# mrluin/TextualDegRemoval

Measured on AMD Instinct MI355X. Metric: train images/sec (512x512, bs=4/GPU), higher is better.
Workload: dtype f32 (3xbf16-split MFMA: 24-bit operand significands on the full fp32 exponent range, fp32 accumulate; unscaled gradients, no loss scale, no step-skip guard; tensors fp32 -- the MASA-encoder ResidualBlock activations / gradients as three bf16 planes whose sum IS the fp32 value, bit for bit)

## Files before the change

### include/tdr.h

```cpp
#ifndef TDR_H
#define TDR_H
#include <stdint.h>
#ifdef __cplusplus
extern "C" {
#endif

#define TDR_ABI_VERSION 109
int tdr_version(void);
const char* tdr_last_error(void);

typedef struct TdrStepGuard {
    float scale, inv_scale, max_scale;
    int good, growth_interval;
    int step, skipped, finite;
    float bc1, bc2_sqrt;
} TdrStepGuard;

typedef struct TdrConvDesc {
    int N, Cin, H, W;
    int Cout, OH, OW;
    int KH, stride, dil, pad;
    const float* in;  int64_t in_ns;
    int gate;
    const float* kscale; int64_t kscale_ns;
// ... 74 lines not shown
    float* g;
    float* db;
    int per_image;
    float* ws; int64_t ws_floats;
    int math;
} TdrWgradDesc;
int64_t tdr_wgrad_ws_floats(const TdrWgradDesc* d);
int tdr_conv_wgrad(const TdrWgradDesc* d, void* stream);

typedef struct TdrWg1GroupEntry {
    const float* in; const float* dout; float* part; float* dbpart; float* g; float* db;
} TdrWg1GroupEntry;
int tdr_wgrad1x1_group_supported(const TdrWgradDesc* d);
int64_t tdr_wgrad1x1_group_ws_floats(const TdrWgradDesc* d, int nprob);
int tdr_wgrad1x1_group(const TdrWgradDesc* d, int nprob, const void* table, void* stream);

int tdr_layernorm2d_fwd(const float* x, int64_t x_ns, const float* w, const float* b, float eps, int center,
                        int N, int C, int HW, float* y, float* mu, float* rstd, void* stream);
int64_t tdr_ln_ws_floats(int N, int C, int HW);
int tdr_layernorm2d_bwd(const float* go, const float* x, int64_t x_ns, const float* mu, const float* rstd,
                        const float* w, const float* add, int64_t add_ns, int add_C, int center,
                        int N, int C, int HW, float* gx, float* gw, float* gb, float* ws, void* stream);

int64_t tdr_dwsg_ws_floats(int N, int C, int H, int W);
int tdr_dwsg_fwd(const float* t, const float* w, const float* b, int N, int C, int H, int W,
                 float* g, float* pooled, float* ws, void* stream);
int tdr_dwsg_bwd(const float* dg, const float* t, const float* w, const float* b, int N, int C, int H, int W,
                 float* dt, float* dw, float* db, float* ws, void* stream);
int tdr_dwsg_bwd_biased(const float* dg, const float* dg_bias, float dg_bias_mul, const float* t, const float* w, const float* b,
                        int N, int C, int H, int W, float* dt, float* dw, float* db, float* ws, void* stream);
// ... 364 lines not shown
```

### textualdegremoval_amd/_lib.py

```python
import ctypes as C
import os

import torch

_HERE = os.path.dirname(os.path.abspath(__file__))
LIB_PATH = os.environ.get('TDR_LIB_PATH', os.path.join(_HERE, 'libtdr_hip.so'))

ABI_VERSION = 109
c_fp = C.c_void_p
i32, i64, f32 = C.c_int, C.c_int64, C.c_float


class TdrConvDesc(C.Structure):
    _fields_ = [
        ('N', i32), ('Cin', i32), ('H', i32), ('W', i32),
        ('Cout', i32), ('OH', i32), ('OW', i32),
        ('KH', i32), ('stride', i32), ('dil', i32), ('pad', i32),
        ('inp', c_fp), ('in_ns', i64),
        ('gate', i32),
        ('kscale', c_fp), ('kscale_ns', i64),
        ('wp', c_fp), ('wp_ns', i64), ('Mpad', i32), ('wp_fmt', i32),
        ('out', c_fp), ('out_ns', i64),
        ('epi', i32),
        ('bias', c_fp), ('bias_ns', i64),
# ... 115 lines not shown
    'tdr_conv3x3_p16_force_cfg': (i32, [i32]),
    'tdr_wgrad3x3_p16_ws_floats': (i64, [C.POINTER(TdrWgradP16Desc)]),
    'tdr_wgrad3x3_p16': (i32, [C.POINTER(TdrWgradP16Desc), c_fp]),
    'tdr_packed_weight_floats': (i64, [i32, i32, i32]),
    'tdr_pack_weights': (i32, [c_fp, i32, i32, i32, i32, c_fp, c_fp]),
    'tdr_packed_weight_bytes_bx3': (i64, [i32, i32, i32]),
    'tdr_pack_weights_bx3': (i32, [c_fp, i32, i32, i32, i32, c_fp, c_fp]),
    'tdr_pack_job_init': (i32, [C.POINTER(TdrPackJob), c_fp, i32, i32, i32, i32, i32, c_fp]),
    'tdr_pack_weights_multi': (i32, [c_fp, i32, i64, c_fp]),
    'tdr_pack_patches': (i32, [c_fp, i32, i32, i32, i32, i32, i32, i32, i32, i32, i32, c_fp, c_fp]),
    'tdr_wgrad_ws_floats': (i64, [C.POINTER(TdrWgradDesc)]),
    'tdr_conv_wgrad': (i32, [C.POINTER(TdrWgradDesc), c_fp]),
    'tdr_wgrad1x1_group_supported': (i32, [C.POINTER(TdrWgradDesc)]),
    'tdr_wgrad1x1_group_ws_floats': (i64, [C.POINTER(TdrWgradDesc), i32]),
    'tdr_wgrad1x1_group': (i32, [C.POINTER(TdrWgradDesc), i32, c_fp, c_fp]),
    'tdr_layernorm2d_fwd': (i32, [c_fp, i64, c_fp, c_fp, f32, i32, i32, i32, i32, c_fp, c_fp, c_fp, c_fp]),
    'tdr_ln_ws_floats': (i64, [i32, i32, i32]),
    'tdr_layernorm2d_bwd': (i32, [c_fp, c_fp, i64, c_fp, c_fp, c_fp, c_fp, i64, i32, i32, i32, i32, i32, c_fp, c_fp, c_fp,
                                  c_fp, c_fp]),
    'tdr_dwsg_ws_floats': (i64, [i32, i32, i32, i32]),
    'tdr_dwsg_fwd': (i32, [c_fp, c_fp, c_fp, i32, i32, i32, i32, c_fp, c_fp, c_fp, c_fp]),
    'tdr_dwsg_bwd': (i32, [c_fp, c_fp, c_fp, c_fp, i32, i32, i32, i32, c_fp, c_fp, c_fp, c_fp, c_fp]),
    'tdr_dwsg_bwd_biased': (i32, [c_fp, c_fp, f32, c_fp, c_fp, c_fp, i32, i32, i32, i32, c_fp, c_fp, c_fp, c_fp, c_fp]),
    'tdr_dwsg_bwd_parts_supported': (i32, [i32]),
    'tdr_dw_param_finish': (i32, [c_fp, i32, i32, i32, i32, c_fp, c_fp, c_fp]),
    'tdr_dwgelu_fwd': (i32, [c_fp, c_fp, c_fp, i32, i32, i32, i32, c_fp, c_fp]),
    'tdr_dwgelu_bwd': (i32, [c_fp, c_fp, c_fp, c_fp, i32, i32, i32, i32, c_fp, c_fp, c_fp, c_fp, c_fp]),
    'tdr_dwconv_fwd': (i32, [c_fp, c_fp, c_fp, i32, i32, i32, i32, c_fp, c_fp]),
    'tdr_dwconv_act_fwd': (i32, [c_fp, c_fp, c_fp, i32, i32, i32, i32, i32, c_fp, c_fp]),
    'tdr_dwconv_act_bwd': (i32, [c_fp, c_fp, c_fp, c_fp, i32, i32, i32, i32, c_fp, c_fp, c_fp, c_fp, c_fp]),
# ... 202 lines not shown
```

### textualdegremoval_amd/csrc/tdr_error.cpp

```cpp
#include <stdarg.h>
#include <stdio.h>
#include "../../include/tdr.h"
static thread_local char g_err[512] = "";
void tdr_set_error(const char* fmt, ...) {
    va_list ap;
    va_start(ap, fmt);
    vsnprintf(g_err, sizeof(g_err), fmt, ap);
    va_end(ap);
}
extern "C" const char* tdr_last_error(void) { return g_err; }
extern "C" int tdr_version(void) { return 109; }
```

### textualdegremoval_amd/csrc/tdr_wgrad_p16.hip

```cpp
#include <stdlib.h>
#include <stdint.h>
#include "tdr_common.h"
#include "../../include/tdr.h"

typedef _Float16 wf16x8 __attribute__((ext_vector_type(8)));
typedef __bf16 wbf16x8 __attribute__((ext_vector_type(8)));
typedef short ws16x4 __attribute__((ext_vector_type(4)));
typedef short ws16x8 __attribute__((ext_vector_type(8)));

namespace {

struct WgP16Args {
    const uint4* in; const uint4* dout;
    int Cin, Cout, H, W, Hp, Wp;
    int strips, chunks, rc;
    float* part; float* dbpart;
};

#define WGP_GLDS(gptr, lptr)                                                                          \
    __builtin_amdgcn_global_load_lds((__attribute__((address_space(1))) const void*)(gptr),          \
                                     (__attribute__((address_space(3))) void*)(lptr), 16, 0, 0)

__device__ __forceinline__ ws16x8 tr_frag(const char* p, int off0, int off1) {
    const ws16x4 a = __builtin_amdgcn_ds_read_tr16_b64_v4i16((__attribute__((address_space(3))) ws16x4*)(p + off0));
    const ws16x4 b = __builtin_amdgcn_ds_read_tr16_b64_v4i16((__attribute__((address_space(3))) ws16x4*)(p + off1));
    const ws16x8 v = {a[0], a[1], a[2], a[3], b[0], b[1], b[2], b[3]};
    return v;
}
template <int NS>
__device__ __forceinline__ f32x16 wg_mfma(ws16x8 x, ws16x8 y, f32x16 c) {
    if constexpr (NS == 3) return __builtin_amdgcn_mfma_f32_32x32x16_bf16(__builtin_bit_cast(wbf16x8, x), __builtin_bit_cast(wbf16x8, y), c, 0, 0, 0);
    else return __builtin_amdgcn_mfma_f32_32x32x16_f16(__builtin_bit_cast(wf16x8, x), __builtin_bit_cast(wf16x8, y), c, 0, 0, 0);
}

template <int WM, int WN, int WK, int NS = 2>
__global__ __launch_bounds__(256, 2) void wgrad3x3_p16_kernel(WgP16Args a) {
    static_assert(WM * WN * WK == 4, "4 waves");
    constexpr int RS = WK == 4 ? 2 : 1;
    static_assert(2 * RS % WK == 0, "k-steps of a step split evenly over the K waves");
    constexpr int BMo = 32 * WM, BNi = 32 * WN, NOo = BMo / 8, NOi = BNi / 8;
    constexpr int XS = 2 * RS + 2, DS = 2 * RS;
    constexpr int XR = ((NOi * NS * 34 + 63) / 64) * 64;
    constexpr int DR = NOo * NS * 32;
    constexpr int XP = XR / 64, DP = DR / 64;

    extern __shared__ __attribute__((aligned(1024))) uint4 smem4[];
    uint4* sX = smem4;
    uint4* sD = smem4 + XS * XR;

    const int tid = threadIdx.x, lane = tid & 63, wave = __builtin_amdgcn_readfirstlane(tid >> 6);
    const int wk = wave % WK, wn = (wave / WK) % WN, wm = wave / (WK * WN);
    int split = blockIdx.x;
    const int chunk = split % a.chunks; int t = split / a.chunks;
    const int strip = t % a.strips;
    const int n = t / a.strips;
    const int co0 = blockIdx.y * BMo, ci0 = blockIdx.z * BNi;
    const int y0 = chunk * a.rc, y1 = min(y0 + a.rc, a.H);
    const int x0 = strip * 32;
    const long PS = (long)a.Hp * a.Wp;
    const int Gi = a.Cin >> 3, Go = a.Cout >> 3;

    constexpr int XPW = (XP + 3) / 4, DPW = (DP + 3) / 4;
    long xoff[XPW], doff[DPW];
    bool dcol[DPW];
#pragma unroll
    for (int i = 0; i < XPW; ++i) {
        const int f = min((wave + 4 * i) * 64 + lane, NOi * NS * 34 - 1);
        const int op = f / 34, c = f - op * 34;
        const int oc = min((ci0 >> 3) + (op / NS), Gi - 1);
        xoff[i] = ((((long)n * Gi + oc) * NS + (op % NS)) * PS + min(x0 + c, a.Wp - 1)) * 16;
    }
#pragma unroll
    for (int i = 0; i < DPW; ++i) {
        const int f = (wave + 4 * i) * 64 + lane;
        const int op = f >> 5, c = f & 31;
        const int oc = min((co0 >> 3) + (op / NS), Go - 1);
        dcol[i] = x0 + c < a.W;
        doff[i] = ((((long)n * Go + oc) * NS + (op % NS)) * PS) * 16;
    }
    const char* xbase = reinterpret_cast<const char*>(a.in);
    const char* dbase = reinterpret_cast<const char*>(a.dout);
    auto glds = [&](const char* src, uint4* dst) {
        const unsigned l = (unsigned)(uintptr_t)(__attribute__((address_space(3))) char*)dst;
        unsigned keep;
        asm volatile("s_mov_b32 %0, m0\n\ts_mov_b32 m0, %2\n\ts_nop 0\n\tglobal_load_lds_dwordx4 %1, off\n\ts_mov_b32 m0, %0"
                     : "=&s"(keep) : "v"(src), "s"(l) : "memory");
    };
    auto issue_x_row = [&](int prow) {
        uint4* dst = sX + (prow % XS) * XR;
        const long rowb = (long)min(prow, a.Hp - 1) * a.Wp * 16;
#pragma unroll
        for (int i = 0; i < XPW; ++i)
            if (wave + 4 * i < XP) glds(xbase + xoff[i] + rowb, dst + (wave + 4 * i) * 64);
    };
    auto issue_d_row = [&](int y) {
        uint4* dst = sD + (y % DS) * DR;
        const bool yok = y < a.H;
        const long rowb = ((long)(y + 1) * a.Wp + x0 + 1) * 16;
#pragma unroll
        for (int i = 0; i < DPW; ++i)
            if (wave + 4 * i < DP) {
                const int c = ((wave + 4 * i) * 64 + lane) & 31;
                glds(dbase + doff[i] + ((yok && dcol[i]) ? rowb + c * 16 : 0), dst + (wave + 4 * i) * 64);
            }
    };

    const int nn = lane & 15, g16 = lane >> 4;
    const int jpx = nn >> 2, q = nn & 3, chalf = g16 & 1, kk = g16 >> 1;
    const int oct = chalf * 2 + (q >> 1);
    const int a_lane = ((wm * 4 + oct) * NS * 32 + 8 * kk + jpx) * 16 + (q & 1) * 8;
    const int b_lane = ((wn * 4 + oct) * NS * 34 + 8 * kk + jpx) * 16 + (q & 1) * 8;

    f32x16 acc[9];
#pragma unroll
    for (int tp = 0; tp < 9; ++tp)
#pragma unroll
        for (int r = 0; r < 16; ++r) acc[tp][r] = 0.f;
    f32x16 accb;
#pragma unroll
    for (int r = 0; r < 16; ++r) accb[r] = 0.f;
    const bool want_db = a.dbpart != nullptr && blockIdx.z == 0 && wn == 0;
    ws16x8 ones;
#pragma unroll
    for (int e = 0; e < 8; ++e) ones[e] = NS == 3 ? (short)0x3f80 : (short)0x3c00;

    issue_x_row(y0); issue_x_row(y0 + 1);
#pragma unroll
    for (int r = 0; r < RS; ++r) { issue_x_row(y0 + 2 + r); issue_d_row(y0 + r); }
    asm volatile("s_waitcnt vmcnt(0) lgkmcnt(0)\n\ts_barrier" ::: "memory");

    for (int y = y0; y < y1; y += RS) {
#pragma unroll
        for (int r = 0; r < RS; ++r) { issue_x_row(y + RS + 2 + r); issue_d_row(y + RS + r); }
#pragma unroll
        for (int u = 0; u < 2 * RS / WK; ++u) {
            const int ku = wk + u * WK;
            const int yr = y + (ku >> 1), ks = ku & 1;
            if (yr < y1) {
                const char* pd = reinterpret_cast<const char*>(sD + (yr % DS) * DR) + a_lane + ks * 256;
                ws16x8 ap[NS];
#pragma unroll
                for (int s = 0; s < NS; ++s) ap[s] = tr_frag(pd, s * 32 * 16, s * 32 * 16 + 64);
                if (want_db) {
#pragma unroll
                    for (int s = NS - 1; s >= 0; --s) accb = wg_mfma<NS>(ap[s], ones, accb);
                }
                constexpr int NPR = NS == 3 ? 6 : 3;
                constexpr int PA[6] = {NS == 3 ? 2 : 1, 0, NS == 3 ? 1 : 0, 1, 0, 0};
                constexpr int PB[6] = {0, NS == 3 ? 2 : 1, NS == 3 ? 1 : 0, 0, 1, 0};
#pragma unroll
                for (int ky = 0; ky < 3; ++ky) {
                    const char* px = reinterpret_cast<const char*>(sX + ((yr + ky) % XS) * XR) + b_lane + ks * 256;
                    ws16x8 bp[NS][3];
#pragma unroll
                    for (int s = 0; s < NS; ++s)
#pragma unroll
                        for (int kx = 0; kx < 3; ++kx) bp[s][kx] = tr_frag(px, s * 34 * 16 + kx * 16, s * 34 * 16 + kx * 16 + 64);
#pragma unroll
                    for (int pr = 0; pr < NPR; ++pr)
#pragma unroll
                        for (int kx = 0; kx < 3; ++kx) acc[ky * 3 + kx] = wg_mfma<NS>(ap[PA[pr]], bp[PB[pr]][kx], acc[ky * 3 + kx]);
                }
            }
        }
        asm volatile("s_waitcnt vmcnt(0) lgkmcnt(0)\n\ts_barrier" ::: "memory");
    }

    const int j = lane & 31, kg = lane >> 5;
    if constexpr (WK > 1) {
        float* red = reinterpret_cast<float*>(smem4);
#pragma unroll
        for (int w = 1; w < WK; ++w) {
            __syncthreads();
            if (wk == w) {
#pragma unroll
                for (int tp = 0; tp < 9; ++tp)
#pragma unroll
                    for (int r = 0; r < 16; ++r) red[(tp * 16 + r) * 64 + lane] = acc[tp][r];
#pragma unroll
                for (int r = 0; r < 16; ++r) red[(9 * 16 + r) * 64 + lane] = accb[r];
// ... 7 lines not shown
#pragma unroll
                for (int r = 0; r < 16; ++r) accb[r] += red[(9 * 16 + r) * 64 + lane];
            }
        }
        if (wk != 0) return;
    }
    float* part = a.part + (long)split * a.Cout * a.Cin * 9;
    const int ci = ci0 + wn * 32 + j;
#pragma unroll
    for (int r = 0; r < 16; ++r) {
        const int co = co0 + wm * 32 + (r & 3) + 8 * (r >> 2) + 4 * kg;
        if (co < a.Cout && ci < a.Cin) {
#pragma unroll
            for (int tp = 0; tp < 9; ++tp) part[((long)co * a.Cin + ci) * 9 + tp] = acc[tp][r];
        }
        if (want_db && j == 0 && co < a.Cout) a.dbpart[(long)split * a.Cout + co] = accb[r];
    }
}

template <int KL>
__global__ __launch_bounds__(64 * KL) void wgrad_p16_reduce_kernel(const float* __restrict__ part, long elems, int nsplit, float* __restrict__ out,
                                                                   int nb_main, const float* __restrict__ part2, long elems2, float* __restrict__ out2) {
    __shared__ float red[KL][64];
    const int lane = threadIdx.x & 63, kl = threadIdx.x >> 6;
    const bool second = (int)blockIdx.x >= nb_main;
    const float* pbase = second ? part2 : part;
    const long ne = second ? elems2 : elems;
    float* o = second ? out2 : out;
    const long e = ((int)blockIdx.x - (second ? nb_main : 0)) * 64L + lane;
    const float* p = pbase + (e < ne ? e : ne - 1);
    float s0 = 0.f;
    for (int k = kl; k < nsplit; k += 8 * KL) {
        float v[8];
#pragma unroll
        for (int u = 0; u < 8; ++u) v[u] = k + u * KL < nsplit ? p[(long)(k + u * KL) * ne] : 0.f;
        s0 += ((v[0] + v[1]) + (v[2] + v[3])) + ((v[4] + v[5]) + (v[6] + v[7]));
    }
    red[kl][lane] = s0;
    __syncthreads();
    if (kl == 0 && e < ne) {
        float t = 0.f;
#pragma unroll
        for (int q = 0; q < KL; ++q) t += red[q][lane];
        o[e] = t;
    }
}

struct WgP16Plan { int cfg, bm, bn, strips, chunks, rc, nsplit; };

WgP16Plan wgp_plan(const TdrWgradP16Desc* d) {
    WgP16Plan p;
    p.cfg = (d->Cin <= 32 && d->Cout <= 32) ? 1 : 0;
    p.bm = p.cfg == 1 ? 32 : 64; p.bn = p.bm;
    const int rs = p.cfg == 1 ? 2 : 1;
    p.strips = tdr_cdiv(d->W, 32);
    const long out_tiles = (long)tdr_cdiv(d->Cout, p.bm) * tdr_cdiv(d->Cin, p.bn);
    static const long want_total = tdr_tune_env("TDR_WGP_WANT") ? atol(tdr_tune_env("TDR_WGP_WANT")) : 512;
    long want = want_total / out_tiles;
    if (want < 1) want = 1;
    const long rows = (long)d->N * p.strips * d->H;
    long rc = (rows + want - 1) / want;
    if (rc < 8) rc = 8;
    rc = (rc + rs - 1) / rs * rs;
    if (rc > d->H) rc = (d->H + rs - 1) / rs * rs;
    p.rc = (int)rc;
    p.chunks = tdr_cdiv(d->H, p.rc);
    p.nsplit = d->N * p.strips * p.chunks;
    return p;
}

template <int WM, int WN, int WK, int NS>
int launch_wgp(const WgP16Args& a, const WgP16Plan& p, const TdrWgradP16Desc* d, hipStream_t st) {
    constexpr int RS = WK == 4 ? 2 : 1, NOo = 4 * WM, NOi = 4 * WN;
    constexpr int XR = ((NOi * NS * 34 + 63) / 64) * 64, DR = NOo * NS * 32;
    size_t lds = (size_t)((2 * RS + 2) * XR + 2 * RS * DR) * 16;
    if (WK > 1 && lds < 10 * 16 * 64 * 4) lds = 10 * 16 * 64 * 4;
    dim3 grid(p.nsplit, tdr_cdiv(d->Cout, 32 * WM), tdr_cdiv(d->Cin, 32 * WN));
    auto kern = wgrad3x3_p16_kernel<WM, WN, WK, NS>;
    static bool attr_set = false;
    if (!attr_set) {
        (void)hipFuncSetAttribute(reinterpret_cast<const void*>(kern), hipFuncAttributeMaxDynamicSharedMemorySize, 160 * 1024);
        attr_set = true;
    }
    hipLaunchKernelGGL(kern, grid, dim3(256), lds, st, a);
    TDR_LAUNCH_CHECK("wgrad3x3_p16_kernel");
    return TDR_OK;
}

}

extern "C" int64_t tdr_wgrad3x3_p16_ws_floats(const TdrWgradP16Desc* d) {
    const WgP16Plan p = wgp_plan(d);
    return (int64_t)p.nsplit * d->Cout * d->Cin * 9 + (int64_t)p.nsplit * d->Cout;
}

extern "C" int tdr_wgrad3x3_p16(const TdrWgradP16Desc* d, void* stream) {
    TDR_REQUIRE(d && d->in16 && d->dout16 && d->g && d->ws, "tdr_wgrad3x3_p16: null pointer");
    TDR_REQUIRE(d->Cin % 16 == 0 && d->Cout % 16 == 0, "tdr_wgrad3x3_p16: channel counts must be multiples of 16 (%d, %d)", d->Cin, d->Cout);
    const WgP16Plan p = wgp_plan(d);
    const int64_t need = tdr_wgrad3x3_p16_ws_floats(d);
    TDR_REQUIRE(d->ws_floats >= need, "tdr_wgrad3x3_p16: workspace too small (%lld < %lld)", (long long)d->ws_floats, (long long)need);
    WgP16Args a;
    a.in = (const uint4*)d->in16; a.dout = (const uint4*)d->dout16;
    a.Cin = d->Cin; a.Cout = d->Cout; a.H = d->H; a.W = d->W; a.Hp = d->H + 2; a.Wp = d->W + 2;
    a.strips = p.strips; a.chunks = p.chunks; a.rc = p.rc;
    a.part = d->ws;
    a.dbpart = d->db ? d->ws + (int64_t)p.nsplit * d->Cout * d->Cin * 9 : nullptr;
    hipStream_t st = (hipStream_t)stream;
    TDR_REQUIRE(d->fmt == 0 || d->fmt == 1 || d->fmt == 2, "tdr_wgrad3x3_p16: plane format %d (1: bf16 triple, 2: fp16 pair)", d->fmt);
    int rc;
    if (d->fmt == 1) rc = p.cfg == 1 ? launch_wgp<1, 1, 4, 3>(a, p, d, st) : launch_wgp<2, 2, 1, 3>(a, p, d, st);
    else rc = p.cfg == 1 ? launch_wgp<1, 1, 4, 2>(a, p, d, st) : launch_wgp<2, 2, 1, 2>(a, p, d, st);
    if (rc != TDR_OK) return rc;
    const long elems = (long)d->Cout * d->Cin * 9;
    const int nb_main = tdr_cdiv(elems, 64), nb2 = d->db ? tdr_cdiv(d->Cout, 64) : 0;
    if (p.nsplit <= 8)
        hipLaunchKernelGGL(wgrad_p16_reduce_kernel<1>, dim3(nb_main + nb2), dim3(64), 0, st, d->ws, elems, p.nsplit, d->g, nb_main, a.dbpart,
                           (long)d->Cout, d->db);
    else if (p.nsplit <= 64)
        hipLaunchKernelGGL(wgrad_p16_reduce_kernel<4>, dim3(nb_main + nb2), dim3(256), 0, st, d->ws, elems, p.nsplit, d->g, nb_main, a.dbpart,
                           (long)d->Cout, d->db);
    else
        hipLaunchKernelGGL(wgrad_p16_reduce_kernel<16>, dim3(nb_main + nb2), dim3(1024), 0, st, d->ws, elems, p.nsplit, d->g, nb_main, a.dbpart,
                           (long)d->Cout, d->db);
    TDR_LAUNCH_CHECK("wgrad_p16_reduce_kernel");
    return TDR_OK;
}
```

### textualdegremoval_amd/engine.py

```python
import contextlib
import os
import types

import torch

from . import kernels as K
from . import leaves as L
from .kernels import (EPI_GATEBWD, EPI_PSHUF, PACK_DGRAD_2X2S2, PACK_DGRAD_3X3S2, PACK_DGRAD_S1, PACK_FWD)

LN_EPS = 1e-6
FUSE_TAIL = True
FUSE_HEAD = True
FUSE_CONV3_DGRAD = True
INFER_KERNELS = True


def _sub(P, pre):
    n = len(pre)
    return {k[n:]: v for k, v in P.items() if k.startswith(pre)}


def _put(G, pre, g):
    for k, v in g.items():
        G[pre + k] = v
# ... 322 lines not shown
    with L.deferred_join():
        _encoder_bwd_levels(dfeats, P, pre, cnt, saved, G, dnext)
    L.maybe_join()
    return None


def _encoder_bwd_levels(dfeats, P, pre, cnt, saved, G, dnext):
    for lvl in reversed(range(len(dfeats))):
        k = lvl + 1
        xin, a, blocks = saved[lvl]
        d = dnext if dnext is not None else dfeats[lvl]
        if d is None:
            continue
        if blocks and isinstance(blocks[0][0], K.P16):
            d16, d32 = K.p16_from_f32(d, fmt=blocks[0][0].fmt), d
            for i in reversed(range(cnt[lvl])):
                bp = f'{pre}blk_L{k}.{i}.'
                x16, h16 = blocks[i]
                w1, w2 = P[bp + 'conv1.weight'], P[bp + 'conv2.weight']
                Cc = w1.shape[0]
                with K.on_side(h16.buf, d16.buf):
                    gw, G[bp + 'conv2.bias'] = K.wgrad3x3_p16(h16, d16, want_db=True)
                    G[bp + 'conv2.weight'] = gw.view(Cc, Cc, 3, 3)
                wp, mp, *_ = K.pack_weights(w2, PACK_DGRAD_S1)
                _, dh16 = K.conv3x3_p16(d16, wp, mp, Cc, mask=h16, want32=False, want16=True)
                with K.on_side(x16.buf, dh16.buf):
                    gw, G[bp + 'conv1.bias'] = K.wgrad3x3_p16(x16, dh16, want_db=True)
                    G[bp + 'conv1.weight'] = gw.view(Cc, Cc, 3, 3)
                wp, mp, *_ = K.pack_weights(w1, PACK_DGRAD_S1)
                first = i == 0
                d32, d16 = K.conv3x3_p16(dh16, wp, mp, Cc, res=d32 if d32 is not None else d16, mask=a if first else None,
                                         want32=first, want16=not first)
            d = d32
        else:
            for i in reversed(range(cnt[lvl])):
                bp = f'{pre}blk_L{k}.{i}.'
                x_in, h = blocks[i]
                w1, w2 = P[bp + 'conv1.weight'], P[bp + 'conv2.weight']
                Cc = w1.shape[0]
                with K.on_side(h, d):
                    gw, G[bp + 'conv2.bias'] = K.conv_wgrad(h, d, Cc, Cc, 3, pad=1, want_db=True)
                    G[bp + 'conv2.weight'] = gw.view(Cc, Cc, 3, 3)
                wp, mp, *_ = K.pack_weights(w2, PACK_DGRAD_S1)
                dh = K.conv_forward(d, wp, mp, Cc, 3, pad=1, mask=h)
                with K.on_side(x_in, dh):
                    gw, G[bp + 'conv1.bias'] = K.conv_wgrad(x_in, dh, Cc, Cc, 3, pad=1, want_db=True)
                    G[bp + 'conv1.weight'] = gw.view(Cc, Cc, 3, 3)
# ... 283 lines not shown
```

### textualdegremoval_amd/kernels.py

```python
import ctypes as C
import os

import torch

from . import _lib
from ._lib import TdrConvDesc, TdrConvP16Desc, TdrWgradDesc, TdrWgradP16Desc, check

EPI_STD, EPI_GATEBWD, EPI_PSHUF = 0, 1, 2
PACK_FWD, PACK_DGRAD_S1, PACK_DGRAD_2X2S2, PACK_DGRAD_3X3S2 = 0, 1, 2, 3

MATH = os.environ.get('TDR_MATH', 'bx3')
WGRAD_1X1_BX3 = True
FMT_F32, FMT_BX3, FMT_HX2, FMT_H1 = 0, 1, 2, 3


def fp16_path():
    return MATH in ('hx2', 'h1')


GRAD_SCALED = False
BACKWARD_PHASE = False


def set_grad_scaled(on):
# ... 658 lines not shown
    bpp = per // (Cout * (Cin + 1))
    ws = workspace(per * n, dev, 'wgrad_group')
    g = torch.empty(n, Cout, Cin, dtype=torch.float32, device=dev)
    db = torch.empty(n, Cout, dtype=torch.float32, device=dev) if want_db else None
    rows = []
    for i, (x, do, *_r) in enumerate(reqs):
        part = ws.data_ptr() + 4 * per * i
        rows += [x.data_ptr(), do.data_ptr(), part, part + 4 * bpp * Cout * Cin if want_db else 0, g.data_ptr() + 4 * Cout * Cin * i,
                 db.data_ptr() + 4 * Cout * i if want_db else 0]
    tab = _upload_table(rows, seq, dev)
    if _survey is not None and d.math >= 2:
        for (_x, do, *_r) in reqs:
            _survey.probe(do, 'grad')
    check(lib.tdr_wgrad1x1_group(C.byref(d), n, tab.data_ptr(), _stream()), 'tdr_wgrad1x1_group')
    return [(g[i].view(1, Cout, Cin, 1, 1), db[i] if want_db else None) for i in range(n)]


def layernorm2d_fwd(x, w, b, eps, center=True):
    lib = _lib.load()
    N, Cc, H, W = x.shape
    y = torch.empty(N, Cc, H, W, dtype=torch.float32, device=x.device)
    mu = torch.empty(N, H * W, dtype=torch.float32, device=x.device)
    rstd = torch.empty_like(mu)
    check(lib.tdr_layernorm2d_fwd(x.data_ptr(), _dense_nchw(x), w.data_ptr(), _p(b), float(eps), 1 if center else 0, N, Cc,
                                  H * W, y.data_ptr(), mu.data_ptr(), rstd.data_ptr(), _stream()), 'tdr_layernorm2d_fwd')
    return y, mu, rstd


def layernorm2d_bwd(go, x, mu, rstd, w, add=None, center=True):
    lib = _lib.load()
# ... 1514 lines not shown
```

Before: 60.36.

## Group encoder ResidualBlock 3x3 weight-gradient kernels into one table-driven launch

Adds a grouped variant of the plane-format 3x3 wgrad kernel. It reads each problem's input, gradient and output pointers from a device table, and each workgroup walks a contiguous range of row/strip work units. The engine defers every conv1/conv2 wgrad in an encoder level and issues them as a single side-stream launch with a grouped split-reduction, instead of one launch per conv. This aims to cut per-launch overhead and fill the GPU better on small per-layer problems. The cost is less interleaving of wgrad with the dgrad chain, plus 32-bit offset arithmetic inside the kernel.

```diff
diff --git a/include/tdr.h b/include/tdr.h
--- a/include/tdr.h
+++ b/include/tdr.h
@@ -5,7 +5,7 @@
 extern "C" {
 #endif
 
-#define TDR_ABI_VERSION 109
+#define TDR_ABI_VERSION 110
 int tdr_version(void);
 const char* tdr_last_error(void);
 
@@ -112,6 +112,10 @@
 int tdr_wgrad1x1_group_supported(const TdrWgradDesc* d);
 int64_t tdr_wgrad1x1_group_ws_floats(const TdrWgradDesc* d, int nprob);
 int tdr_wgrad1x1_group(const TdrWgradDesc* d, int nprob, const void* table, void* stream);
+
+int64_t tdr_wgrad3x3_p16_group_ws_floats(const TdrWgradP16Desc* d, int nprob);
+int tdr_wgrad3x3_p16_group_plan(const TdrWgradP16Desc* d, int nprob, int* nsplit, int* units, int* units_per_wg);
+int tdr_wgrad3x3_p16_group(const TdrWgradP16Desc* d, int nprob, const void* table, void* stream);
 
 int tdr_layernorm2d_fwd(const float* x, int64_t x_ns, const float* w, const float* b, float eps, int center,
                         int N, int C, int HW, float* y, float* mu, float* rstd, void* stream);
diff --git a/textualdegremoval_amd/_lib.py b/textualdegremoval_amd/_lib.py
--- a/textualdegremoval_amd/_lib.py
+++ b/textualdegremoval_amd/_lib.py
@@ -6,7 +6,7 @@
 _HERE = os.path.dirname(os.path.abspath(__file__))
 LIB_PATH = os.environ.get('TDR_LIB_PATH', os.path.join(_HERE, 'libtdr_hip.so'))
 
-ABI_VERSION = 109
+ABI_VERSION = 110
 c_fp = C.c_void_p
 i32, i64, f32 = C.c_int, C.c_int64, C.c_float
 
@@ -153,6 +153,9 @@
     'tdr_wgrad1x1_group_supported': (i32, [C.POINTER(TdrWgradDesc)]),
     'tdr_wgrad1x1_group_ws_floats': (i64, [C.POINTER(TdrWgradDesc), i32]),
     'tdr_wgrad1x1_group': (i32, [C.POINTER(TdrWgradDesc), i32, c_fp, c_fp]),
+    'tdr_wgrad3x3_p16_group_ws_floats': (i64, [C.POINTER(TdrWgradP16Desc), i32]),
+    'tdr_wgrad3x3_p16_group_plan': (i32, [C.POINTER(TdrWgradP16Desc), i32, C.POINTER(i32), C.POINTER(i32), C.POINTER(i32)]),
+    'tdr_wgrad3x3_p16_group': (i32, [C.POINTER(TdrWgradP16Desc), i32, c_fp, c_fp]),
     'tdr_layernorm2d_fwd': (i32, [c_fp, i64, c_fp, c_fp, f32, i32, i32, i32, i32, c_fp, c_fp, c_fp, c_fp]),
     'tdr_ln_ws_floats': (i64, [i32, i32, i32]),
     'tdr_layernorm2d_bwd': (i32, [c_fp, c_fp, i64, c_fp, c_fp, c_fp, c_fp, i64, i32, i32, i32, i32, i32, c_fp, c_fp, c_fp,
diff --git a/textualdegremoval_amd/csrc/tdr_error.cpp b/textualdegremoval_amd/csrc/tdr_error.cpp
--- a/textualdegremoval_amd/csrc/tdr_error.cpp
+++ b/textualdegremoval_amd/csrc/tdr_error.cpp
@@ -9,4 +9,4 @@
     va_end(ap);
 }
 extern "C" const char* tdr_last_error(void) { return g_err; }
-extern "C" int tdr_version(void) { return 109; }
+extern "C" int tdr_version(void) { return 110; }
diff --git a/textualdegremoval_amd/csrc/tdr_wgrad_p16.hip b/textualdegremoval_amd/csrc/tdr_wgrad_p16.hip
--- a/textualdegremoval_amd/csrc/tdr_wgrad_p16.hip
+++ b/textualdegremoval_amd/csrc/tdr_wgrad_p16.hip
@@ -15,6 +15,7 @@
     int Cin, Cout, H, W, Hp, Wp;
     int strips, chunks, rc;
     float* part; float* dbpart;
+    const void* grp_tab; int grp_pairs, grp_nsplit, grp_units, tiles_co, tiles_ci;
 };
 
 #define WGP_GLDS(gptr, lptr)                                                                          \
@@ -33,7 +34,7 @@
     else return __builtin_amdgcn_mfma_f32_32x32x16_f16(__builtin_bit_cast(wf16x8, x), __builtin_bit_cast(wf16x8, y), c, 0, 0, 0);
 }
 
-template <int WM, int WN, int WK, int NS = 2>
+template <int WM, int WN, int WK, int NS = 2, bool GRP = false>
 __global__ __launch_bounds__(256, 2) void wgrad3x3_p16_kernel(WgP16Args a) {
     static_assert(WM * WN * WK == 4, "4 waves");
     constexpr int RS = WK == 4 ? 2 : 1;
@@ -50,60 +51,29 @@
 
     const int tid = threadIdx.x, lane = tid & 63, wave = __builtin_amdgcn_readfirstlane(tid >> 6);
     const int wk = wave % WK, wn = (wave / WK) % WN, wm = wave / (WK * WN);
-    int split = blockIdx.x;
-    const int chunk = split % a.chunks; int t = split / a.chunks;
-    const int strip = t % a.strips;
-    const int n = t / a.strips;
-    const int co0 = blockIdx.y * BMo, ci0 = blockIdx.z * BNi;
-    const int y0 = chunk * a.rc, y1 = min(y0 + a.rc, a.H);
-    const int x0 = strip * 32;
+    int split = blockIdx.x, u0 = blockIdx.x, u1 = u0 + 1, tco = blockIdx.y, tci = blockIdx.z;
+    float* dbout = a.dbpart;
+    if constexpr (GRP) {
+        const int T = a.tiles_co * a.tiles_ci;
+        const int c8 = (int)blockIdx.x / (8 * T), r = (int)blockIdx.x - c8 * (8 * T);
+        const int pair = c8 * 8 + (r & 7), tile = r >> 3;
+        if (pair >= a.grp_pairs) return;
+        const int prob = pair / a.grp_nsplit;
+        split = pair - prob * a.grp_nsplit;
+        tco = tile % a.tiles_co; tci = tile / a.tiles_co;
+        u0 = (int)((long)split * a.grp_units / a.grp_nsplit);
+        u1 = (int)((long)(split + 1) * a.grp_units / a.grp_nsplit);
+        const TdrWg1GroupEntry e = static_cast<const TdrWg1GroupEntry*>(a.grp_tab)[prob];
+        a.in = reinterpret_cast<const uint4*>(e.in); a.dout = reinterpret_cast<const uint4*>(e.dout);
+        const bool direct = a.grp_nsplit == 1;
+        a.part = direct ? e.g : e.part;
+        dbout = direct ? e.db : e.dbpart;
+    }
+    const int co0 = tco * BMo, ci0 = tci * BNi;
     const long PS = (long)a.Hp * a.Wp;
     const int Gi = a.Cin >> 3, Go = a.Cout >> 3;
-
-    constexpr int XPW = (XP + 3) / 4, DPW = (DP + 3) / 4;
-    long xoff[XPW], doff[DPW];
-    bool dcol[DPW];
-#pragma unroll
-    for (int i = 0; i < XPW; ++i) {
-        const int f = min((wave + 4 * i) * 64 + lane, NOi * NS * 34 - 1);
-        const int op = f / 34, c = f - op * 34;
-        const int oc = min((ci0 >> 3) + (op / NS), Gi - 1);
-        xoff[i] = ((((long)n * Gi + oc) * NS + (op % NS)) * PS + min(x0 + c, a.Wp - 1)) * 16;
-    }
-#pragma unroll
-    for (int i = 0; i < DPW; ++i) {
-        const int f = (wave + 4 * i) * 64 + lane;
-        const int op = f >> 5, c = f & 31;
-        const int oc = min((co0 >> 3) + (op / NS), Go - 1);
-        dcol[i] = x0 + c < a.W;
-        doff[i] = ((((long)n * Go + oc) * NS + (op % NS)) * PS) * 16;
-    }
     const char* xbase = reinterpret_cast<const char*>(a.in);
     const char* dbase = reinterpret_cast<const char*>(a.dout);
-    auto glds = [&](const char* src, uint4* dst) {
-        const unsigned l = (unsigned)(uintptr_t)(__attribute__((address_space(3))) char*)dst;
-        unsigned keep;
-        asm volatile("s_mov_b32 %0, m0\n\ts_mov_b32 m0, %2\n\ts_nop 0\n\tglobal_load_lds_dwordx4 %1, off\n\ts_mov_b32 m0, %0"
-                     : "=&s"(keep) : "v"(src), "s"(l) : "memory");
-    };
-    auto issue_x_row = [&](int prow) {
-        uint4* dst = sX + (prow % XS) * XR;
-        const long rowb = (long)min(prow, a.Hp - 1) * a.Wp * 16;
-#pragma unroll
-        for (int i = 0; i < XPW; ++i)
-            if (wave + 4 * i < XP) glds(xbase + xoff[i] + rowb, dst + (wave + 4 * i) * 64);
-    };
-    auto issue_d_row = [&](int y) {
-        uint4* dst = sD + (y % DS) * DR;
-        const bool yok = y < a.H;
-        const long rowb = ((long)(y + 1) * a.Wp + x0 + 1) * 16;
-#pragma unroll
-        for (int i = 0; i < DPW; ++i)
-            if (wave + 4 * i < DP) {
-                const int c = ((wave + 4 * i) * 64 + lane) & 31;
-                glds(dbase + doff[i] + ((yok && dcol[i]) ? rowb + c * 16 : 0), dst + (wave + 4 * i) * 64);
-            }
-    };
 
     const int nn = lane & 15, g16 = lane >> 4;
     const int jpx = nn >> 2, q = nn & 3, chalf = g16 & 1, kk = g16 >> 1;
@@ -119,51 +89,104 @@
     f32x16 accb;
 #pragma unroll
     for (int r = 0; r < 16; ++r) accb[r] = 0.f;
-    const bool want_db = a.dbpart != nullptr && blockIdx.z == 0 && wn == 0;
+    const bool want_db = dbout != nullptr && tci == 0 && wn == 0;
     ws16x8 ones;
 #pragma unroll
     for (int e = 0; e < 8; ++e) ones[e] = NS == 3 ? (short)0x3f80 : (short)0x3c00;
 
-    issue_x_row(y0); issue_x_row(y0 + 1);
-#pragma unroll
-    for (int r = 0; r < RS; ++r) { issue_x_row(y0 + 2 + r); issue_d_row(y0 + r); }
-    asm volatile("s_waitcnt vmcnt(0) lgkmcnt(0)\n\ts_barrier" ::: "memory");
-
-    for (int y = y0; y < y1; y += RS) {
-#pragma unroll
-        for (int r = 0; r < RS; ++r) { issue_x_row(y + RS + 2 + r); issue_d_row(y + RS + r); }
-#pragma unroll
-        for (int u = 0; u < 2 * RS / WK; ++u) {
-            const int ku = wk + u * WK;
-            const int yr = y + (ku >> 1), ks = ku & 1;
-            if (yr < y1) {
-                const char* pd = reinterpret_cast<const char*>(sD + (yr % DS) * DR) + a_lane + ks * 256;
-                ws16x8 ap[NS];
-#pragma unroll
-                for (int s = 0; s < NS; ++s) ap[s] = tr_frag(pd, s * 32 * 16, s * 32 * 16 + 64);
-                if (want_db) {
-#pragma unroll
-                    for (int s = NS - 1; s >= 0; --s) accb = wg_mfma<NS>(ap[s], ones, accb);
+    for (int u = u0; u < u1; ++u) {
+        const int chunk = u % a.chunks; const int t = u / a.chunks;
+        const int strip = t % a.strips;
+        const int n = t / a.strips;
+        const int y0 = chunk * a.rc, y1 = min(y0 + a.rc, a.H);
+        const int x0 = strip * 32;
+
+        constexpr int XPW = (XP + 3) / 4, DPW = (DP + 3) / 4;
+        unsigned xoff[XPW], doff[DPW];
+        const char* xb = xbase + (long)n * Gi * NS * PS * 16;
+        const char* db = dbase + (long)n * Go * NS * PS * 16;
+        bool dcol[DPW];
+#pragma unroll
+        for (int i = 0; i < XPW; ++i) {
+            const int f = min((wave + 4 * i) * 64 + lane, NOi * NS * 34 - 1);
+            const int op = f / 34, c = f - op * 34;
+            const int oc = min((ci0 >> 3) + (op / NS), Gi - 1);
+            xoff[i] = (unsigned)((((long)oc * NS + (op % NS)) * PS + min(x0 + c, a.Wp - 1)) * 16);
+        }
+#pragma unroll
+        for (int i = 0; i < DPW; ++i) {
+            const int f = (wave + 4 * i) * 64 + lane;
+            const int op = f >> 5, c = f & 31;
+            const int oc = min((co0 >> 3) + (op / NS), Go - 1);
+            dcol[i] = x0 + c < a.W;
+            doff[i] = (unsigned)((((long)oc * NS + (op % NS)) * PS) * 16);
+        }
+        auto glds = [&](const char* base, unsigned off, uint4* dst) {
+            const unsigned l = (unsigned)(uintptr_t)(__attribute__((address_space(3))) char*)dst;
+            unsigned keep;
+            asm volatile("s_mov_b32 %0, m0\n\ts_mov_b32 m0, %2\n\ts_nop 0\n\tglobal_load_lds_dwordx4 %1, %3\n\ts_mov_b32 m0, %0"
+                         : "=&s"(keep) : "v"(off), "s"(l), "s"(base) : "memory");
+        };
+        auto issue_x_row = [&](int prow) {
+            uint4* dst = sX + (prow % XS) * XR;
+            const long rowb = (long)min(prow, a.Hp - 1) * a.Wp * 16;
+#pragma unroll
+            for (int i = 0; i < XPW; ++i)
+                if (wave + 4 * i < XP) glds(xb + rowb, xoff[i], dst + (wave + 4 * i) * 64);
+        };
+        auto issue_d_row = [&](int y) {
+            uint4* dst = sD + (y % DS) * DR;
+            const bool yok = y < a.H;
+            const unsigned rowb = (unsigned)(((long)(y + 1) * a.Wp + x0 + 1) * 16);
+#pragma unroll
+            for (int i = 0; i < DPW; ++i)
+                if (wave + 4 * i < DP) {
+                    const int c = ((wave + 4 * i) * 64 + lane) & 31;
+                    glds(db, doff[i] + ((yok && dcol[i]) ? rowb + c * 16 : 0u), dst + (wave + 4 * i) * 64);
                 }
-                constexpr int NPR = NS == 3 ? 6 : 3;
-                constexpr int PA[6] = {NS == 3 ? 2 : 1, 0, NS == 3 ? 1 : 0, 1, 0, 0};
-                constexpr int PB[6] = {0, NS == 3 ? 2 : 1, NS == 3 ? 1 : 0, 0, 1, 0};
-#pragma unroll
-                for (int ky = 0; ky < 3; ++ky) {
-                    const char* px = reinterpret_cast<const char*>(sX + ((yr + ky) % XS) * XR) + b_lane + ks * 256;
-                    ws16x8 bp[NS][3];
-#pragma unroll
-                    for (int s = 0; s < NS; ++s)
-#pragma unroll
-                        for (int kx = 0; kx < 3; ++kx) bp[s][kx] = tr_frag(px, s * 34 * 16 + kx * 16, s * 34 * 16 + kx * 16 + 64);
-#pragma unroll
-                    for (int pr = 0; pr < NPR; ++pr)
-#pragma unroll
-                        for (int kx = 0; kx < 3; ++kx) acc[ky * 3 + kx] = wg_mfma<NS>(ap[PA[pr]], bp[PB[pr]][kx], acc[ky * 3 + kx]);
+        };
+
+        issue_x_row(y0); issue_x_row(y0 + 1);
+#pragma unroll
+        for (int r = 0; r < RS; ++r) { issue_x_row(y0 + 2 + r); issue_d_row(y0 + r); }
+        asm volatile("s_waitcnt vmcnt(0) lgkmcnt(0)\n\ts_barrier" ::: "memory");
+
+        for (int y = y0; y < y1; y += RS) {
+#pragma unroll
+            for (int r = 0; r < RS; ++r) { issue_x_row(y + RS + 2 + r); issue_d_row(y + RS + r); }
+#pragma unroll
+            for (int uu = 0; uu < 2 * RS / WK; ++uu) {
+                const int ku = wk + uu * WK;
+                const int yr = y + (ku >> 1), ks = ku & 1;
+                if (yr < y1) {
+                    const char* pd = reinterpret_cast<const char*>(sD + (yr % DS) * DR) + a_lane + ks * 256;
+                    ws16x8 ap[NS];
+#pragma unroll
+                    for (int s = 0; s < NS; ++s) ap[s] = tr_frag(pd, s * 32 * 16, s * 32 * 16 + 64);
+                    if (want_db) {
+#pragma unroll
+                        for (int s = NS - 1; s >= 0; --s) accb = wg_mfma<NS>(ap[s], ones, accb);
+                    }
+                    constexpr int NPR = NS == 3 ? 6 : 3;
+                    constexpr int PA[6] = {NS == 3 ? 2 : 1, 0, NS == 3 ? 1 : 0, 1, 0, 0};
+                    constexpr int PB[6] = {0, NS == 3 ? 2 : 1, NS == 3 ? 1 : 0, 0, 1, 0};
+#pragma unroll
+                    for (int ky = 0; ky < 3; ++ky) {
+                        const char* px = reinterpret_cast<const char*>(sX + ((yr + ky) % XS) * XR) + b_lane + ks * 256;
+                        ws16x8 bp[NS][3];
+#pragma unroll
+                        for (int s = 0; s < NS; ++s)
+#pragma unroll
+                            for (int kx = 0; kx < 3; ++kx) bp[s][kx] = tr_frag(px, s * 34 * 16 + kx * 16, s * 34 * 16 + kx * 16 + 64);
+#pragma unroll
+                        for (int pr = 0; pr < NPR; ++pr)
+#pragma unroll
+                            for (int kx = 0; kx < 3; ++kx) acc[ky * 3 + kx] = wg_mfma<NS>(ap[PA[pr]], bp[PB[pr]][kx], acc[ky * 3 + kx]);
+                    }
                 }
             }
+            asm volatile("s_waitcnt vmcnt(0) lgkmcnt(0)\n\ts_barrier" ::: "memory");
         }
-        asm volatile("s_waitcnt vmcnt(0) lgkmcnt(0)\n\ts_barrier" ::: "memory");
     }
 
     const int j = lane & 31, kg = lane >> 5;
@@ -201,20 +224,20 @@
 #pragma unroll
             for (int tp = 0; tp < 9; ++tp) part[((long)co * a.Cin + ci) * 9 + tp] = acc[tp][r];
         }
-        if (want_db && j == 0 && co < a.Cout) a.dbpart[(long)split * a.Cout + co] = accb[r];
+        if (want_db && j == 0 && co < a.Cout) dbout[(long)split * a.Cout + co] = accb[r];
     }
 }
 
 template <int KL>
-__global__ __launch_bounds__(64 * KL) void wgrad_p16_reduce_kernel(const float* __restrict__ part, long elems, int nsplit, float* __restrict__ out,
-                                                                   int nb_main, const float* __restrict__ part2, long elems2, float* __restrict__ out2) {
+__device__ __forceinline__ void wgp_reduce_block(const float* __restrict__ part, long elems, int nsplit, float* __restrict__ out, int nb_main,
+                                                 const float* __restrict__ part2, long elems2, float* __restrict__ out2, int bx) {
     __shared__ float red[KL][64];
     const int lane = threadIdx.x & 63, kl = threadIdx.x >> 6;
-    const bool second = (int)blockIdx.x >= nb_main;
+    const bool second = bx >= nb_main;
     const float* pbase = second ? part2 : part;
     const long ne = second ? elems2 : elems;
     float* o = second ? out2 : out;
-    const long e = ((int)blockIdx.x - (second ? nb_main : 0)) * 64L + lane;
+    const long e = (bx - (second ? nb_main : 0)) * 64L + lane;
     const float* p = pbase + (e < ne ? e : ne - 1);
     float s0 = 0.f;
     for (int k = kl; k < nsplit; k += 8 * KL) {
@@ -233,17 +256,33 @@
     }
 }
 
+template <int KL>
+__global__ __launch_bounds__(64 * KL) void wgrad_p16_reduce_kernel(const float* __restrict__ part, long elems, int nsplit, float* __restrict__ out,
+                                                                   int nb_main, const float* __restrict__ part2, long elems2, float* __restrict__ out2) {
+    wgp_reduce_block<KL>(part, elems, nsplit, out, nb_main, part2, elems2, out2, (int)blockIdx.x);
+}
+
+template <int KL>
+__global__ __launch_bounds__(64 * KL) void wgrad_p16_reduce_kernel_grp(const TdrWg1GroupEntry* __restrict__ tab, long elems, int nsplit, int Cout,
+                                                                       int nb_main) {
+    const TdrWg1GroupEntry e = tab[blockIdx.y];
+    if ((int)blockIdx.x >= nb_main && (e.db == nullptr || e.dbpart == nullptr)) return;
+    wgp_reduce_block<KL>(e.part, elems, nsplit, e.g, nb_main, e.dbpart, (long)Cout, e.db, (int)blockIdx.x);
+}
+
 struct WgP16Plan { int cfg, bm, bn, strips, chunks, rc, nsplit; };
 
-WgP16Plan wgp_plan(const TdrWgradP16Desc* d) {
+long wgp_want_total() {
+    static const long want_total = tdr_tune_env("TDR_WGP_WANT") ? atol(tdr_tune_env("TDR_WGP_WANT")) : 512;
+    return want_total;
+}
+
+WgP16Plan wgp_plan_for(const TdrWgradP16Desc* d, long want) {
     WgP16Plan p;
     p.cfg = (d->Cin <= 32 && d->Cout <= 32) ? 1 : 0;
     p.bm = p.cfg == 1 ? 32 : 64; p.bn = p.bm;
     const int rs = p.cfg == 1 ? 2 : 1;
     p.strips = tdr_cdiv(d->W, 32);
-    const long out_tiles = (long)tdr_cdiv(d->Cout, p.bm) * tdr_cdiv(d->Cin, p.bn);
-    static const long want_total = tdr_tune_env("TDR_WGP_WANT") ? atol(tdr_tune_env("TDR_WGP_WANT")) : 512;
-    long want = want_total / out_tiles;
     if (want < 1) want = 1;
     const long rows = (long)d->N * p.strips * d->H;
     long rc = (rows + want - 1) / want;
@@ -256,21 +295,46 @@
     return p;
 }
 
-template <int WM, int WN, int WK, int NS>
+bool wgp_image_fits(const TdrWgradP16Desc* d) {
+    const long c = d->Cin > d->Cout ? d->Cin : d->Cout;
+    return c / 8 * 3 * (long)(d->H + 2) * (d->W + 2) * 16 < (1L << 32);
+}
+
+long wgp_out_tiles(const TdrWgradP16Desc* d) {
+    const int t = (d->Cin <= 32 && d->Cout <= 32) ? 32 : 64;
+    return (long)tdr_cdiv(d->Cout, t) * tdr_cdiv(d->Cin, t);
+}
+
+WgP16Plan wgp_plan(const TdrWgradP16Desc* d) { return wgp_plan_for(d, wgp_want_total() / wgp_out_tiles(d)); }
+
+struct WgP16GroupPlan { WgP16Plan p; int units, nsplit; };
+
+WgP16GroupPlan wgp_group_plan(const TdrWgradP16Desc* d, int nprob) {
+    WgP16GroupPlan gp;
+    long want = wgp_want_total() / ((long)nprob * wgp_out_tiles(d));
+    if (want < 1) want = 1;
+    gp.p = wgp_plan_for(d, want);
+    gp.units = gp.p.nsplit;
+    gp.nsplit = (int)(want < gp.units ? want : gp.units);
+    return gp;
+}
+
+template <int WM, int WN, int WK, int NS, bool GRP = false>
 int launch_wgp(const WgP16Args& a, const WgP16Plan& p, const TdrWgradP16Desc* d, hipStream_t st) {
     constexpr int RS = WK == 4 ? 2 : 1, NOo = 4 * WM, NOi = 4 * WN;
     constexpr int XR = ((NOi * NS * 34 + 63) / 64) * 64, DR = NOo * NS * 32;
     size_t lds = (size_t)((2 * RS + 2) * XR + 2 * RS * DR) * 16;
     if (WK > 1 && lds < 10 * 16 * 64 * 4) lds = 10 * 16 * 64 * 4;
     dim3 grid(p.nsplit, tdr_cdiv(d->Cout, 32 * WM), tdr_cdiv(d->Cin, 32 * WN));
-    auto kern = wgrad3x3_p16_kernel<WM, WN, WK, NS>;
+    if (GRP) grid = dim3((unsigned)tdr_cdiv(a.grp_pairs, 8) * 8 * a.tiles_co * a.tiles_ci);
+    auto kern = wgrad3x3_p16_kernel<WM, WN, WK, NS, GRP>;
     static bool attr_set = false;
     if (!attr_set) {
         (void)hipFuncSetAttribute(reinterpret_cast<const void*>(kern), hipFuncAttributeMaxDynamicSharedMemorySize, 160 * 1024);
         attr_set = true;
     }
     hipLaunchKernelGGL(kern, grid, dim3(256), lds, st, a);
-    TDR_LAUNCH_CHECK("wgrad3x3_p16_kernel");
+    TDR_LAUNCH_CHECK(GRP ? "wgrad3x3_p16_kernel<grouped>" : "wgrad3x3_p16_kernel");
     return TDR_OK;
 }
 
@@ -284,6 +348,7 @@
 extern "C" int tdr_wgrad3x3_p16(const TdrWgradP16Desc* d, void* stream) {
     TDR_REQUIRE(d && d->in16 && d->dout16 && d->g && d->ws, "tdr_wgrad3x3_p16: null pointer");
     TDR_REQUIRE(d->Cin % 16 == 0 && d->Cout % 16 == 0, "tdr_wgrad3x3_p16: channel counts must be multiples of 16 (%d, %d)", d->Cin, d->Cout);
+    TDR_REQUIRE(wgp_image_fits(d), "tdr_wgrad3x3_p16: a plane image of more than 4 GiB");
     const WgP16Plan p = wgp_plan(d);
     const int64_t need = tdr_wgrad3x3_p16_ws_floats(d);
     TDR_REQUIRE(d->ws_floats >= need, "tdr_wgrad3x3_p16: workspace too small (%lld < %lld)", (long long)d->ws_floats, (long long)need);
@@ -292,6 +357,7 @@
     a.Cin = d->Cin; a.Cout = d->Cout; a.H = d->H; a.W = d->W; a.Hp = d->H + 2; a.Wp = d->W + 2;
     a.strips = p.strips; a.chunks = p.chunks; a.rc = p.rc;
     a.part = d->ws;
+    a.grp_tab = nullptr; a.grp_pairs = a.grp_nsplit = a.grp_units = a.tiles_co = a.tiles_ci = 0;
     a.dbpart = d->db ? d->ws + (int64_t)p.nsplit * d->Cout * d->Cin * 9 : nullptr;
     hipStream_t st = (hipStream_t)stream;
     TDR_REQUIRE(d->fmt == 0 || d->fmt == 1 || d->fmt == 2, "tdr_wgrad3x3_p16: plane format %d (1: bf16 triple, 2: fp16 pair)", d->fmt);
@@ -313,3 +379,53 @@
     TDR_LAUNCH_CHECK("wgrad_p16_reduce_kernel");
     return TDR_OK;
 }
+
+extern "C" int64_t tdr_wgrad3x3_p16_group_ws_floats(const TdrWgradP16Desc* d, int nprob) {
+    if (!d || nprob < 1) return 0;
+    const WgP16GroupPlan gp = wgp_group_plan(d, nprob);
+    if (gp.nsplit == 1) return 0;
+    return (int64_t)gp.nsplit * d->Cout * d->Cin * 9 + (int64_t)gp.nsplit * d->Cout;
+}
+
+extern "C" int tdr_wgrad3x3_p16_group_plan(const TdrWgradP16Desc* d, int nprob, int* nsplit, int* units, int* units_per_wg) {
+    TDR_REQUIRE(d && nprob > 0, "tdr_wgrad3x3_p16_group_plan: null argument");
+    const WgP16GroupPlan gp = wgp_group_plan(d, nprob);
+    if (nsplit) *nsplit = gp.nsplit;
+    if (units) *units = gp.units;
+    if (units_per_wg) *units_per_wg = tdr_cdiv(gp.units, gp.nsplit);
+    return TDR_OK;
+}
+
+extern "C" int tdr_wgrad3x3_p16_group(const TdrWgradP16Desc* d, int nprob, const void* table, void* stream) {
+    TDR_REQUIRE(d && table && nprob > 0, "tdr_wgrad3x3_p16_group: null argument");
+    TDR_REQUIRE(d->Cin % 16 == 0 && d->Cout % 16 == 0, "tdr_wgrad3x3_p16_group: channel counts must be multiples of 16 (%d, %d)", d->Cin, d->Cout);
+    TDR_REQUIRE(d->fmt == 0 || d->fmt == 1 || d->fmt == 2, "tdr_wgrad3x3_p16_group: plane format %d (1: bf16 triple, 2: fp16 pair)", d->fmt);
+    TDR_REQUIRE(wgp_image_fits(d), "tdr_wgrad3x3_p16_group: a plane image of more than 4 GiB");
+    const WgP16GroupPlan gp = wgp_group_plan(d, nprob);
+    const WgP16Plan& p = gp.p;
+    WgP16Args a;
+    a.in = nullptr; a.dout = nullptr; a.part = nullptr; a.dbpart = nullptr;
+    a.Cin = d->Cin; a.Cout = d->Cout; a.H = d->H; a.W = d->W; a.Hp = d->H + 2; a.Wp = d->W + 2;
+    a.strips = p.strips; a.chunks = p.chunks; a.rc = p.rc;
+    a.grp_tab = table; a.grp_nsplit = gp.nsplit; a.grp_units = gp.units;
+    a.tiles_co = tdr_cdiv(d->Cout, p.bm); a.tiles_ci = tdr_cdiv(d->Cin, p.bn);
+    const long pairs = (long)nprob * gp.nsplit;
+    TDR_REQUIRE(pairs * a.tiles_co * a.tiles_ci < (1L << 30), "tdr_wgrad3x3_p16_group: too many workgroups (%ld pairs)", pairs);
+    a.grp_pairs = (int)pairs;
+    hipStream_t st = (hipStream_t)stream;
+    int rc;
+    if (d->fmt == 1) rc = p.cfg == 1 ? launch_wgp<1, 1, 4, 3, true>(a, p, d, st) : launch_wgp<2, 2, 1, 3, true>(a, p, d, st);
+    else rc = p.cfg == 1 ? launch_wgp<1, 1, 4, 2, true>(a, p, d, st) : launch_wgp<2, 2, 1, 2, true>(a, p, d, st);
+    if (rc != TDR_OK || gp.nsplit == 1) return rc;
+    const long elems = (long)d->Cout * d->Cin * 9;
+    const int nb_main = tdr_cdiv(elems, 64), nb2 = tdr_cdiv(d->Cout, 64);
+    const TdrWg1GroupEntry* tab = static_cast<const TdrWg1GroupEntry*>(table);
+    if (gp.nsplit <= 8)
+        hipLaunchKernelGGL(wgrad_p16_reduce_kernel_grp<1>, dim3(nb_main + nb2, nprob), dim3(64), 0, st, tab, elems, gp.nsplit, d->Cout, nb_main);
+    else if (gp.nsplit <= 64)
+        hipLaunchKernelGGL(wgrad_p16_reduce_kernel_grp<4>, dim3(nb_main + nb2, nprob), dim3(256), 0, st, tab, elems, gp.nsplit, d->Cout, nb_main);
+    else
+        hipLaunchKernelGGL(wgrad_p16_reduce_kernel_grp<16>, dim3(nb_main + nb2, nprob), dim3(1024), 0, st, tab, elems, gp.nsplit, d->Cout, nb_main);
+    TDR_LAUNCH_CHECK("wgrad_p16_reduce_kernel_grp");
+    return TDR_OK;
+}
diff --git a/textualdegremoval_amd/engine.py b/textualdegremoval_amd/engine.py
--- a/textualdegremoval_amd/engine.py
+++ b/textualdegremoval_amd/engine.py
@@ -360,23 +360,39 @@
             continue
         if blocks and isinstance(blocks[0][0], K.P16):
             d16, d32 = K.p16_from_f32(d, fmt=blocks[0][0].fmt), d
+            fmts = {t.fmt for bl in blocks for t in bl} | {d16.fmt}
+            grouped = GROUP_LEAVES and 2 * cnt[lvl] > 1 and len(fmts) == 1
+            late = []
             for i in reversed(range(cnt[lvl])):
                 bp = f'{pre}blk_L{k}.{i}.'
                 x16, h16 = blocks[i]
                 w1, w2 = P[bp + 'conv1.weight'], P[bp + 'conv2.weight']
                 Cc = w1.shape[0]
-                with K.on_side(h16.buf, d16.buf):
-                    gw, G[bp + 'conv2.bias'] = K.wgrad3x3_p16(h16, d16, want_db=True)
-                    G[bp + 'conv2.weight'] = gw.view(Cc, Cc, 3, 3)
+                if grouped:
+                    late.append((bp + 'conv2', h16, d16))
+                else:
+                    with K.on_side(h16.buf, d16.buf):
+                        gw, G[bp + 'conv2.bias'] = K.wgrad3x3_p16(h16, d16, want_db=True)
+                        G[bp + 'conv2.weight'] = gw.view(Cc, Cc, 3, 3)
                 wp, mp, *_ = K.pack_weights(w2, PACK_DGRAD_S1)
                 _, dh16 = K.conv3x3_p16(d16, wp, mp, Cc, mask=h16, want32=False, want16=True)
-                with K.on_side(x16.buf, dh16.buf):
-                    gw, G[bp + 'conv1.bias'] = K.wgrad3x3_p16(x16, dh16, want_db=True)
-                    G[bp + 'conv1.weight'] = gw.view(Cc, Cc, 3, 3)
+                if grouped:
+                    late.append((bp + 'conv1', x16, dh16))
+                else:
+                    with K.on_side(x16.buf, dh16.buf):
+                        gw, G[bp + 'conv1.bias'] = K.wgrad3x3_p16(x16, dh16, want_db=True)
+                        G[bp + 'conv1.weight'] = gw.view(Cc, Cc, 3, 3)
                 wp, mp, *_ = K.pack_weights(w1, PACK_DGRAD_S1)
                 first = i == 0
                 d32, d16 = K.conv3x3_p16(dh16, wp, mp, Cc, res=d32 if d32 is not None else d16, mask=a if first else None,
                                          want32=first, want16=not first)
+            if late:
+                with K.on_side(*[t.buf for _, x16, g16 in late for t in (x16, g16)]):
+                    res = K.wgrad3x3_p16_group([(x16, g16) for _, x16, g16 in late], seq=('enc3x3', pre, lvl), want_db=True)
+                    for (name, x16, g16), (gw, gb) in zip(late, res):
+                        G[name + '.bias'] = gb
+                        G[name + '.weight'] = gw.view(g16.C, x16.C, 3, 3)
+                late.clear()
             d = d32
         else:
             for i in reversed(range(cnt[lvl])):
diff --git a/textualdegremoval_amd/kernels.py b/textualdegremoval_amd/kernels.py
--- a/textualdegremoval_amd/kernels.py
+++ b/textualdegremoval_amd/kernels.py
@@ -1,3 +1,4 @@
+import contextlib
 import ctypes as C
 import os
 
@@ -696,6 +697,45 @@
             _survey.probe(do, 'grad')
     check(lib.tdr_wgrad1x1_group(C.byref(d), n, tab.data_ptr(), _stream()), 'tdr_wgrad1x1_group')
     return [(g[i].view(1, Cout, Cin, 1, 1), db[i] if want_db else None) for i in range(n)]
+
+
+def _wgrad3x3_p16_group_desc(x16, d16):
+    d = TdrWgradP16Desc()
+    d.N, d.Cin, d.H, d.W, d.Cout = x16.N, x16.C, x16.H, x16.W, d16.C
+    d.fmt = x16.fmt
+    return d
+
+
+def wgrad3x3_p16_group_plan(x16, d16, nprob):
+    d = _wgrad3x3_p16_group_desc(x16, d16)
+    ns, un, upw = C.c_int(), C.c_int(), C.c_int()
+    check(_lib.load().tdr_wgrad3x3_p16_group_plan(C.byref(d), nprob, C.byref(ns), C.byref(un), C.byref(upw)), 'tdr_wgrad3x3_p16_group_plan')
+    return ns.value, un.value, upw.value
+
+
+def wgrad3x3_p16_group(reqs, seq, want_db=True):
+    lib = _lib.load()
+    x0, d0 = reqs[0]
+    assert all((x.N, x.C, x.H, x.W, x.fmt, do.C, do.fmt) == (x0.N, x0.C, x0.H, x0.W, x0.fmt, d0.C, x0.fmt) and (do.N, do.H, do.W) == (x.N, x.H, x.W)
+               for x, do in reqs), 'wgrad3x3_p16_group: one shape and plane format per group'
+    dev = x0.buf.device
+    n, Cin, Cout = len(reqs), x0.C, d0.C
+    d = _wgrad3x3_p16_group_desc(x0, d0)
+    per = int(lib.tdr_wgrad3x3_p16_group_ws_floats(C.byref(d), n))
+    nsplit = per // (Cout * (Cin * 9 + 1))
+    ws = workspace(per * n, dev, 'wgrad_group') if per else None
+    g = torch.empty(n, Cout, Cin, 3, 3, dtype=torch.float32, device=dev)
+    db = torch.empty(n, Cout, dtype=torch.float32, device=dev) if want_db else None
+    rows = []
+    for i, (x, do) in enumerate(reqs):
+        part = ws.data_ptr() + 4 * per * i if per else 0
+        rows += [x.data_ptr(), do.data_ptr(), part, part + 4 * nsplit * Cout * Cin * 9 if (want_db and per) else 0, g.data_ptr() + 4 * Cout * Cin * 9 * i,
+                 db.data_ptr() + 4 * Cout * i if want_db else 0]
+    with torch.cuda.stream(_side_stream) if _side_active else contextlib.nullcontext():
+        tab = _upload_table(rows, seq, dev)
+    side_keep(tab)
+    check(lib.tdr_wgrad3x3_p16_group(C.byref(d), n, tab.data_ptr(), _stream()), 'tdr_wgrad3x3_p16_group')
+    return [(g[i].view(1, Cout, Cin, 3, 3), db[i] if want_db else None) for i in range(n)]
 
 
 def layernorm2d_fwd(x, w, b, eps, center=True):
```

New measurement: 61.42 (median of 6 runs). 1.02x the previous value.
